# langfod/Zonos

Hardware: AMD Instinct MI355X
Metric: audio-sec/sec (RTF), Zonos-v0.1-transformer AR decode loop + DAC decode (higher is better)
Workload: dtype bf16; 1 GPU; Zonos-v0.1-transformer bf16, batch=1 per GPU, 10 s target audio (861 frames, 868 decode steps + prefill of 25 positions, EOS suppressed), greedy, cfg_scale 2; weights=seeded synthetic (zonos_amd/synth.py), parallelism=dp1 (utterance sharding, no data-path collective)

## Files before the change

### zonos_amd/csrc/zn_api.hip

```cpp
#include "../../include/zonos_hip.h"
#include "zn_decode_kernels.h"
#include "zn_chain_kernel.h"
#include "zn_step_kernel.h"
#include "zn_prefill_kernels.h"
#include "zn_cond_kernels.h"
#include "zn_mamba_kernels.h"

#include <cmath>
#include <cstdio>
#include <cstdlib>
#include <cstring>
#include <mutex>
#include <string>
#include <vector>

static thread_local std::string g_create_err;
#define ZN_GRAPH_STEPS 8
#define ZN_G16_PART_BYTES ((size_t)8 << 20)
#define ZN_REARM_AFTER 4

struct StepPlan {
  enum Path { LAUNCHES, CHAIN, STACK } path = LAUNCHES;
  int nbk = 0;
  int attn_fused = 0;
// ... 536 lines not shown
struct PostAttnPlans { LinearPlan out, fc1; };
static PostAttnPlans plan_post_attention(zn_handle h, int rows) {
  const zn_config& c = h->cfg;
  const LinearEnv e = linear_env(h);
  PostAttnPlans pp;
  pp.out = plan_linear(e, PRO_NONE, EPI_RESID, rows, c.d_model, c.n_heads * h->hd, h->tune[ZN_TUNE_WG_OUT_PROJ], false, true, false);
  pp.fc1 = plan_linear(e, PRO_LN, EPI_SILU, rows, 2 * c.d_ff, c.d_model, h->tune[ZN_TUNE_WG_FC1], false, false, pp.out.writes_ln_stats);
  return pp;
}

static int layer_in_proj(zn_handle h, int li, bf16_t* x, bf16_t* kv, int max_len, const int* lengths, int rows, hipStream_t s) {
  return run_gemv<PRO_LN, EPI_ROPE_KV>(h, in_proj_args(h, h->layers[li], x, kv, max_len, lengths), rows, h->tune[ZN_TUNE_WG_IN_PROJ], s);
}

static int layer_post_attention(zn_handle h, int li, bf16_t* x, int rows, hipStream_t s, bf16_t* x1_copy = nullptr) {
  const zn_layer_weights& lw = h->layers[li];
  const PostAttnPlans pp = plan_post_attention(h, rows);
  int rc;
  GemvArgs o = out_proj_args(h, lw, h->o1, x, x);
  o.ln_part_out = h->ln_part;
  if (h->cfg.double_out_proj) {
    if ((rc = run_gemv<PRO_NONE, EPI_STORE>(h, out_proj_args(h, lw, h->o1, h->q, nullptr), rows, h->tune[ZN_TUNE_WG_OUT_PROJ], s))) return rc;
    o.x = h->q;
  }
  if ((rc = launch_linear<PRO_NONE, EPI_RESID>(h, pp.out, o, rows, s))) return rc;
  if (x1_copy) (void)hipMemcpyAsync(x1_copy, x, (size_t)rows * h->cfg.d_model * 2, hipMemcpyDeviceToDevice, s);
  if ((rc = launch_linear<PRO_LN, EPI_SILU>(h, pp.fc1, fc1_args(h, lw, x, pp.out.writes_ln_stats ? h->ln_part : nullptr), rows, s))) return rc;
  return run_gemv<PRO_NONE, EPI_RESID>(h, fc2_args(h, lw, x), rows, h->tune[ZN_TUNE_WG_FC2], s);
}

static int layer_decode(zn_handle h, int li, bf16_t* x, bf16_t* kv, int max_len, const int* lengths, const int* ext,
                        int ext_scalar, int rows, int attn_fused, hipStream_t s) {
  int rc;
  if ((rc = layer_in_proj(h, li, x, kv, max_len, lengths, rows, s))) return rc;
  if ((rc = run_attention(h, h->q, kv, max_len, lengths, ext, ext_scalar, h->o1, rows, attn_fused, s))) return rc;
  return layer_post_attention(h, li, x, rows, s);
}

static bf16_t* chain_x(zn_handle h, int li) { return (li & 1) ? h->ch_x2 : h->x; }

static bool chain_heads_fit(zn_handle h) {
  const int units = (h->cfg.n_codebooks * h->cfg.vocab_head + 1) / 2, ppw = (units + ZN_CH_GRID - 1) / ZN_CH_GRID;
  return ppw <= ZN_CH_CWAVES * 5 && ppw * 2 <= 64;
}

static int launch_chain(zn_handle h, int li, const std::vector<const void*>& kv_layers, int max_len, const int* lengths, hipStream_t s,
                        const bf16_t* xin = nullptr, bool with_heads = false) {
  const zn_config& c = h->cfg;
  const zn_layer_weights& lw = h->layers[li];
  const bool last = li + 1 >= c.n_layer;
  ChainArgs a{};
  a.W_out = (const bf16_t*)lw.out_proj; a.W_fc1 = (const bf16_t*)lw.fc1; a.W_fc2 = (const bf16_t*)lw.fc2;
  a.ln2_w = (const bf16_t*)lw.norm2_w; a.ln2_b = (const bf16_t*)lw.norm2_b; a.eps = c.norm_eps; a.F = c.d_ff;
  a.a = h->o1; a.xin = xin ? xin : chain_x(h, li); a.xout = chain_x(h, li + 1);
  a.g_y1 = h->ch_gy1; a.g_x1 = h->ch_gx1; a.g_x2 = h->ch_gx2; a.g_m = h->ch_gm;
  a.epoch = h->ch_epoch; a.tmo = &h->st->pad[0]; a.diag = h->ch_diag;
  a.dbg_pause = h->dbg_pause; a.stamp_layer = li;
  a.stamps = h->ch_stamps ? h->ch_stamps + (size_t)li * 32 : nullptr;
  if (!last) {
    const zn_layer_weights& nx = h->layers[li + 1];
    a.W_in = (const bf16_t*)nx.in_proj; a.lnn_w = (const bf16_t*)nx.norm_w; a.lnn_b = (const bf16_t*)nx.norm_b;
    a.nqkv = (c.n_heads + 2 * c.n_heads_kv) * h->hd;
    a.q_out = h->q; a.kv = (bf16_t*)kv_layers[li + 1]; a.rope = h->rope; a.lengths = lengths;
    a.max_len = max_len; a.hd = h->hd; a.n_heads = c.n_heads; a.n_heads_kv = c.n_heads_kv; a.rope_positions = c.rope_positions;
  }
  const bool heads = last && with_heads;
  if (heads) {
    a.W_in = (const bf16_t*)h->heads; a.lnn_w = (const bf16_t*)h->norm_f_w; a.lnn_b = (const bf16_t*)h->norm_f_b;
    a.nqkv = c.n_codebooks * c.vocab_head; a.heads_out = h->logits_raw;
  }
  const dim3 grid(ZN_CH_GRID), block(ZN_CH_THREADS);
  if (h->ch_variant == 1) {
    if (heads) hipLaunchKernelGGL((chain_kernel<4, 1, 8, 4, 5>), grid, block, ZN_CH_DYN_LDS, s, a);
    else if (last) hipLaunchKernelGGL((chain_kernel<4, 1, 8, 4, 0>), grid, block, ZN_CH_DYN_LDS, s, a);
    else hipLaunchKernelGGL((chain_kernel<4, 1, 8, 4, 2>), grid, block, ZN_CH_DYN_LDS, s, a);
  } else {
    if (heads) hipLaunchKernelGGL((chain_kernel<1, 1, 2, 1, 5>), grid, block, ZN_CH_DYN_LDS, s, a);
    else if (last) hipLaunchKernelGGL((chain_kernel<1, 1, 2, 1, 0>), grid, block, ZN_CH_DYN_LDS, s, a);
    else hipLaunchKernelGGL((chain_kernel<1, 1, 2, 1, 1>), grid, block, ZN_CH_DYN_LDS, s, a);
  }
  return ZN_OK;
}

#define ZN_SK_T1 4, 2, 10, 5, 6, 6
#define ZN_SK_T2 4, 2, 11, 6, 7, 8
#define ZN_SK_T3 4, 2, 13, 7, 8, 12
static int stack_variant_of(int mode) { return mode <= 6 ? 1 : mode <= 8 ? 2 : 3; }
template <int R, int NCH, int T_OUT, int T_FC1, int T_FC2, int T_IN, int NBV>
static bool stack_variant_ok(zn_handle h, int natt) {
  const zn_config& c = h->cfg;
  const int nsw = ZN_CH_GRID - natt;
  if (nsw < 64) return false;
  auto most = [&](int units) { return (units + nsw - 1) / nsw; };
  const int nqkv = (c.n_heads + 2 * c.n_heads_kv) * h->hd;
  const int p_out = most(c.d_model / 2), p_fc1 = 2 * most(c.d_ff / 2), p_qkv = most((nqkv + 1) / 2), p_hd = most((c.n_codebooks * c.vocab_head + 1) / 2);
  if (p_out > ZN_SK_CW * T_OUT || p_out > T_FC2 || p_fc1 > ZN_SK_CW * T_FC1 || p_qkv > ZN_SK_CW * T_IN || p_hd > ZN_SK_CW * T_IN) return false;
  if (p_qkv > 10) return false;
  if (p_out * 2 > 64 || p_out * 4 > 64 || p_fc1 > 64 || p_qkv * 2 > 64 || p_hd * 2 > 64 || nqkv % 2) return false;
  const void* fn = R == 1 ? (const void*)step_r1_kernel<NCH, T_OUT, T_FC1, T_FC2, T_IN, NBV> : (const void*)step_kernel<NCH, T_OUT, T_FC1, T_FC2, T_IN, NBV>;
  int dev = 0, n_cus = 0, per_cu = 0;
  if (hipGetDevice(&dev) != hipSuccess || hipDeviceGetAttribute(&n_cus, hipDeviceAttributeMultiprocessorCount, dev) != hipSuccess) { (void)hipGetLastError(); return false; }
  if (hipFuncSetAttribute(fn, hipFuncAttributeMaxDynamicSharedMemorySize, ZN_SK_DYN_LDS) != hipSuccess) { (void)hipGetLastError(); return false; }
  if (hipOccupancyMaxActiveBlocksPerMultiprocessor(&per_cu, fn, ZN_SK_THREADS, ZN_SK_DYN_LDS) != hipSuccess) { (void)hipGetLastError(); return false; }
  hipFuncAttributes fa{};
  if (hipFuncGetAttributes(&fa, fn) != hipSuccess) { (void)hipGetLastError(); return false; }
  return per_cu >= 1 && n_cus >= ZN_CH_GRID && fa.localSizeBytes == 0;
}
static bool stack_shapes_ok(zn_handle h) {
  const zn_config& c = h->cfg;
  if (h->ch_variant != 1 || h->hd != 128 || c.n_heads_kv < 1 || c.n_heads != 4 * c.n_heads_kv) return false;
  const int npairs = 2 * c.n_heads_kv, nkvh = c.n_heads_kv;
  h->stackv_ok[1] = stack_variant_ok<2, ZN_SK_T1>(h, npairs * 6);
  h->stackv_ok[2] = stack_variant_ok<2, ZN_SK_T2>(h, npairs * 8);
  h->stackv_ok[3] = stack_variant_ok<2, ZN_SK_T3>(h, npairs * ZN_SK_KB_MAXNB);
  h->stackv1_ok[1] = stack_variant_ok<1, ZN_SK_T1>(h, nkvh * 6);
  h->stackv1_ok[2] = stack_variant_ok<1, ZN_SK_T2>(h, nkvh * 8);
  h->stackv1_ok[3] = stack_variant_ok<1, ZN_SK_T3>(h, nkvh * ZN_SK_KB_MAXNB);
  h->stack1_ok = h->stackv1_ok[1];
  return h->stackv_ok[1];
}
static bool persist_allowed(zn_handle h) { return h->tune[ZN_TUNE_PERSISTENT] != 2 && !h->demoted && h->persist_ok && !h->rows_unequal2 && !h->prefix_set; }
static bool persist_shape(zn_handle h, int rows) { return h->ch_variant != 0 && (rows == 2 || (rows == 1 && h->ch_variant == 1)); }
static bool persist_active(zn_handle h, int rows) { return persist_shape(h, rows) && persist_allowed(h); }
static int stack_blocks_for(zn_handle h, int rows, int keys_upper_bound) {
  if (h->tune[ZN_TUNE_WHOLE_STEP] == 2 || !(rows == 1 ? h->stack1_ok : h->stack_ok)) return -1;
  const int nb = keys_upper_bound <= 512 ? 1 : (keys_upper_bound + 511) / 512;
  return nb <= ZN_SK_KB_MAXNB && (rows == 1 ? h->stackv1_ok : h->stackv_ok)[stack_variant_of(nb)] ? nb : -1;
}
static int graph_slot_for(const StepPlan& p) { return p.path == StepPlan::STACK ? 8 + (p.run > 1 ? ZN_SK_KB_MAXNB + 1 : 0) + p.nbk : p.attn_fused + (p.run > 1 ? 4 : 0); }
static bool chain_allowed(zn_handle h, int rows) { return h->ch_variant != 0 && rows == 2 && persist_allowed(h); }
static StepPlan plan_blocks(zn_handle h, int rows, int keys) {
  StepPlan p;
  p.path = chain_allowed(h, rows) ? StepPlan::CHAIN : StepPlan::LAUNCHES; p.attn_fused = attn_fused_for(h, keys);
  return p;
}
static StepPlan plan_steps(zn_handle h, int steps_left) {
  const int rows = h->rows, keys = h->len_hi + 1, keys_run = h->len_hi + ZN_GRAPH_STEPS;
  const bool want_run = steps_left >= ZN_GRAPH_STEPS && h->tune[ZN_TUNE_GRAPH_RUNS] > 1;
  const bool tail_ok = h->cfg.arch == 0 && persist_active(h, rows) && h->batch <= 2;
  const int nb_run = tail_ok && want_run ? stack_blocks_for(h, rows, keys_run) : -1;
  const int nb_one = tail_ok ? stack_blocks_for(h, rows, keys) : -1;
  StepPlan p = plan_blocks(h, rows, keys);
  if (nb_run >= 0 || nb_one >= 0) {
    p.path = StepPlan::STACK; p.nbk = nb_run >= 0 ? nb_run : nb_one; p.run = nb_run >= 0 ? ZN_GRAPH_STEPS : 1;
  } else if (want_run && attn_fused_for(h, keys_run) == p.attn_fused) p.run = ZN_GRAPH_STEPS;
  p.fused_tail = tail_ok && p.path != StepPlan::LAUNCHES;
  p.graph_slot = graph_slot_for(p);
  return p;
}
static bool stack_pre(zn_handle h) { return h->tune[ZN_TUNE_STACK_PRE] != 2; }
static int launch_stack(zn_handle h, hipStream_t s, int rows, int nbk) {
  const zn_config& c = h->cfg;
  ChainArgs a{};
  a.eps = c.norm_eps; a.F = c.d_ff; a.nqkv = (c.n_heads + 2 * c.n_heads_kv) * h->hd;
  a.xin = h->x_emb; a.xout = h->x;
  a.g_y1 = h->ch_gy1; a.g_x1 = h->ch_gx1; a.g_x2 = h->ch_gx2; a.g_m = h->ch_gm; a.g_qkv = h->ch_gqkv; a.g_a = h->ch_ga;
  a.g_bmax = h->ch_gbmax; a.g_part = h->ch_gpart;
  a.epoch = h->ch_epoch; a.tmo = &h->st->pad[0]; a.diag = h->ch_diag;
  a.dbg_pause = h->dbg_pause;
  a.stamps = h->ch_stamps; a.stamp_layer = c.n_layer / 2;
  a.rope = h->rope; a.lengths = h->lengths; a.max_len = h->max_len; a.hd = h->hd; a.n_heads = c.n_heads; a.n_heads_kv = c.n_heads_kv;
  a.rope_positions = c.rope_positions;
  a.layers = h->stack_layers; a.n_layer = c.n_layer; a.q0 = h->q; a.scale = (float)(1.0 / std::sqrt((double)h->hd));
  a.heads_rows = c.n_codebooks * c.vocab_head; a.heads_out = h->logits_raw; a.trace = h->dbg_trace;
  const int mode = nbk, npairs = rows * c.n_heads_kv;
  a.natt = npairs * (mode < 1 ? 1 : mode);
  if (stack_pre(h)) {
    a.pre_W = (const bf16_t*)h->layers[0].in_proj; a.pre_ln_w = (const bf16_t*)h->layers[0].norm_w; a.pre_ln_b = (const bf16_t*)h->layers[0].norm_b;
    a.pre_kv = (bf16_t*)h->kv_layers[0];
  }
  const dim3 grid(ZN_CH_GRID), block(ZN_SK_THREADS);
  if (rows == 1) {
    switch (stack_variant_of(mode)) {
      case 1: hipLaunchKernelGGL((step_r1_kernel<ZN_SK_T1>), grid, block, ZN_SK_DYN_LDS, s, a); break;
      case 2: hipLaunchKernelGGL((step_r1_kernel<ZN_SK_T2>), grid, block, ZN_SK_DYN_LDS, s, a); break;
      default: hipLaunchKernelGGL((step_r1_kernel<ZN_SK_T3>), grid, block, ZN_SK_DYN_LDS, s, a); break;
    }
    return ZN_OK;
  }
// ... 1088 lines not shown
```

### zonos_amd/csrc/zn_step_kernel.h

```cpp
#pragma once
#include "zn_chain_kernel.h"
#include "zn_step_sched.h"

#define ZN_SK_THREADS 512
#define ZN_SK_CW 4
#ifndef ZN_SK_NBUF
#define ZN_SK_NBUF 3
#endif
#ifndef ZN_SK_PARK
#define ZN_SK_PARK 4
#endif
#ifndef ZN_SK_HELP
#define ZN_SK_HELP 0
#endif
#ifndef ZN_SK_HELP_AT
#define ZN_SK_HELP_AT 0
#endif
#ifndef ZN_SK_EARLY
#define ZN_SK_EARLY 0
#endif
#ifndef ZN_SK_MSWEEP_DELAY
#define ZN_SK_MSWEEP_DELAY 0
#endif
#ifndef ZN_SK_SWEEP_DELAY
#define ZN_SK_SWEEP_DELAY 32
#endif
#define ZN_SK_DYN_LDS (ZN_SK_CW * ZN_SK_PARK * 8192)
#ifndef ZN_SK_APOLL
#define ZN_SK_APOLL 1
#endif
#ifndef ZN_SK_XDELAY
#define ZN_SK_XDELAY 16
#endif
#ifndef ZN_SK_XDELAY_NB
#define ZN_SK_XDELAY_NB 5
#endif
#ifndef ZN_SK_PACE_MARGIN
#define ZN_SK_PACE_MARGIN 0
#endif
#ifndef ZN_SK_PACE_SHIFT
#define ZN_SK_PACE_SHIFT 2
#endif

#ifndef ZN_SK_PACE_CAP
#define ZN_SK_PACE_CAP 8192u
#endif
#define ZN_SK_LONG_WAIT 20000u
struct StepPacer {
  unsigned long long t_ref; unsigned prev;
  unsigned worst = 0, n_long = 0;
  ZN_DEVINL void start() { t_ref = __builtin_amdgcn_s_memrealtime(); }
  ZN_DEVINL void sleep() const {
#ifdef ZN_TIMING_STREAM_ONLY
    return;
#endif
    const unsigned long long until = t_ref + (ZN_SK_PACE_MARGIN > 0 ? (prev > ZN_SK_PACE_MARGIN ? prev - ZN_SK_PACE_MARGIN : 0u) : (prev - (prev >> ZN_SK_PACE_SHIFT)));
    while (__builtin_amdgcn_s_memrealtime() < until) __builtin_amdgcn_s_sleep(8);
  }
  ZN_DEVINL void done() {
    const unsigned long long d = __builtin_amdgcn_s_memrealtime() - t_ref;
    prev = d < ZN_SK_PACE_CAP ? (unsigned)d : ZN_SK_PACE_CAP;
    const unsigned du = d < 0xffffffffull ? (unsigned)d : 0xffffffffu;
    worst = du > worst ? du : worst;
    n_long += du > ZN_SK_LONG_WAIT ? 1u : 0u;
  }
  ZN_DEVINL void report(unsigned* diag, int lane) const {
    if (lane == 0 && diag) { if (worst > ZN_SK_LONG_WAIT / 2) atomicMax(diag + 8, worst); if (n_long) atomicAdd(diag + 9, n_long); }
  }
};
ZN_DEVINL void step_debug_pause(unsigned ticks) {
  const unsigned long long t0 = __builtin_amdgcn_s_memrealtime();
  while (__builtin_amdgcn_s_memrealtime() - t0 < ticks) __builtin_amdgcn_s_sleep(127);
}

#define ZN_SK_KB_MAXNB 12
#define ZN_SK_KB_PSZ 520
struct StepKbLds {
  float sc[4][512];
  float bm[8][4];
  float bmall[ZN_SK_KB_MAXNB][4];
  float accw[8][4][128];
  float l[8][4];
  __attribute__((aligned(16))) bf16_t p[4][512];
  __attribute__((aligned(16))) bf16_t q[4][128];
  __attribute__((aligned(16))) bf16_t knew[128], vnew[128];
  __attribute__((aligned(16))) bf16_t out[4][128];
};
static_assert(sizeof(StepKbLds) <= ZN_SK_DYN_LDS, "the key-block attention role's LDS fits the launch's dynamic LDS");

template <int CH, int DEPTH>
ZN_DEVINL void kb_combine_chunk(__amdgpu_buffer_rsrc_t rs_part, int voff, int loff, int j0, int nb, unsigned tag, const float (*bmall)[4], int g,
                                float& tot0, float& tot1, float& lt, float& mprev, int* tmo, int lane, SweepWho who) {
  constexpr int PSZ8 = ZN_SK_KB_PSZ * 8;
  u32x4 pv[DEPTH][CH];
  u32x2 pl[DEPTH][CH];
  auto issue = [&](auto DC) {
    constexpr int d = decltype(DC)::value;
#pragma unroll
    for (int j = 0; j < CH; ++j) {
      const int jo = min(j0 + j, nb - 1) * PSZ8;
      pv[d][j] = ld_sc1_16(rs_part, voff + jo);
      pl[d][j] = ld_sc1_8(rs_part, loff + jo);
    }
  };
  zn_static_for<0, DEPTH>([&](auto DC) { issue(DC); });
  SpinBound sb; sb.begin();
  int got = -1;
  while (got < 0) {
    zn_static_for<0, DEPTH>([&](auto DC) {
      constexpr int d = decltype(DC)::value;
// ... 212 lines not shown
      const int g = tid >> 7, d = tid & 127;
      float v = 0.f, l = 0.f;
#pragma unroll
      for (int w = 0; w < NW; ++w) v += S.accw[w][g][d];
#pragma unroll
      for (int w = 0; w < NW; ++w) l += S.l[w][g];
      if (nb == 1) S.out[g][d] = f2bf(__fmul_rn(v, 1.0f / l));
      else {
        unsigned long long* pp = a.g_part + ((size_t)pair * MAXNB + jb) * PSZ;
        st_granule(pp + g * 128 + d, tag, __float_as_uint(v));
        if (d == 0) st_granule(pp + G * 128 + g, tag, __float_as_uint(l));
      }
    }
    if (nb == 1) __syncthreads();
    stamp(5);
    if (wave < 4 && (nb == 1 || jb == 0)) {
      const int p = tid, g = p >> 6, dp = p & 63;
      unsigned o;
      if (nb == 1) o = *(const unsigned*)&S.out[g][2 * dp];
      else {
        const int voff = ((pair * MAXNB) * PSZ + g * 128 + 2 * dp) * 8, loff = ((pair * MAXNB) * PSZ + G * 128 + g) * 8;
        float tot0 = 0.f, tot1 = 0.f, lt = 0.f, mprev = -INFINITY;
        const SweepWho who{(8u << 8) | (unsigned)li, a.diag};
        if (ZN_SK_XDELAY > 0 && nb >= ZN_SK_XDELAY_NB) __builtin_amdgcn_s_sleep(ZN_SK_XDELAY);
        if (nb <= 2) kb_combine_chunk<2, ZN_SK_APOLL>(rs_part, voff, loff, 0, nb, tag, S.bmall, g, tot0, tot1, lt, mprev, a.tmo, lane, who);
        else if (nb <= 4) kb_combine_chunk<4, 2>(rs_part, voff, loff, 0, nb, tag, S.bmall, g, tot0, tot1, lt, mprev, a.tmo, lane, who);
        else {
#pragma unroll
          for (int j0 = 0; j0 < NBV; j0 += 6)
            if (j0 < nb) kb_combine_chunk<6, 1>(rs_part, voff, loff, j0, nb, tag, S.bmall, g, tot0, tot1, lt, mprev, a.tmo, lane, who);
        }
        const float inv = 1.0f / lt;
        o = pack2(__fmul_rn(tot0, inv), __fmul_rn(tot1, inv));
      }
      st_granule(a.g_a + (size_t)ar * (D / 2) + ((kvh * G + g) * HD) / 2 + dp, tag, o);
      if (a.trace) *(unsigned*)(a.trace + ((size_t)(8 * li + 1) * R + ar) * D + (kvh * G + g) * HD + 2 * dp) = o;
    }
    if (a.trace && jb == 0 && wave == ZN_SK_CW)
      *(u32x4*)(a.trace + ((size_t)(8 * li + 2) * R + ar) * D + (kvh * G + (lane >> 4)) * HD + (lane & 15) * 8) = *(const u32x4*)&S.q[lane >> 4][(lane & 15) * 8];
    stamp(6);
    if (li + 1 < a.n_layer) {
      int opq = 0;
      asm volatile("" : "+v"(opq));
      issue_kv(a.layers[li + 1].kv, opq, lane);
    }
    pace.start();
  }
  if (wave == ZN_SK_CW) pace.report(a.diag, lane_in);
}

template <int R, int NCH, int T_OUT, int T_FC1, int T_FC2, int T_IN, int NBV>
ZN_DEVINL void step_body(const ChainArgs& a) {
  static_assert(R == 1 || R == 2, "one or two activation rows");
  constexpr int D = NCH * 512, CW = ZN_SK_CW;
  constexpr int NS = 2 * T_OUT + T_FC1 + T_FC2 + T_IN;
  constexpr int NOPS = 5;
  constexpr int MASK = ZN_CH_DEFER_MASK;
  constexpr int NB = ZN_SK_NBUF, P = ZN_SK_PARK;
  constexpr int NL = NS - T_OUT;
  static_assert(T_IN > 0 && NCH == 4, "step_kernel: d_model 2048, head size 128");
  static_assert(P >= T_OUT && NB >= 2 && P + NB <= NL, "op 0's tiles are parked (op 1 reads them again); the prefetch stays inside the block");
  const int tid = threadIdx.x, lane = tid & 63, wave = __builtin_amdgcn_readfirstlane(tid >> 6);
  const int c = blockIdx.x;
  const int F = a.F;
  const unsigned tag0 = ld_sc1_u32(a.epoch);
  extern __shared__ __attribute__((aligned(16))) unsigned char zn_dyn_lds[];
  const int natt = a.natt;
  if (c < natt) {
    step_attention_kb_role<NBV, R>(a, *reinterpret_cast<StepKbLds*>(zn_dyn_lds), tag0, c, wave, lane);
    return;
  }
  __shared__ __attribute__((aligned(16))) bf16_t s_act[R * D];
  __shared__ float s_res[2][64][2][R];
  __shared__ __attribute__((aligned(16))) bf16_t s_ln[4 * D];
  const int sc = c - natt, NSW = (int)gridDim.x - natt;
  auto split = [&](int U, int& n, int& start) { const int base = U / NSW, extra = U % NSW; n = base + (sc < extra ? 1 : 0); start = sc * base + min(sc, extra); };
  int n_out, s_out, ng1, sg1;
  split(D / 2, n_out, s_out);
  split(F / 2, ng1, sg1);
  const int n_fc1 = 2 * ng1, s_fc1 = 2 * sg1;
  int n_qkv, s_qkv, n_hd, s_hd;
  split((a.nqkv + 1) / 2, n_qkv, s_qkv);
  split((a.heads_rows + 1) / 2, n_hd, s_hd);
  constexpr int NBAR = 14;
  __shared__ int s_pf[2];
  constexpr int NPT = 5;
  const bool pre = a.pre_W != nullptr;
  if (tid < 2) s_pf[tid] = 0;
  __syncthreads();

  using SC = StepSched<T_OUT, T_FC1, T_FC2, T_IN, NB, P, ZN_SK_HELP, MASK, ZN_SK_EARLY>;
  auto op_of = [](int s) constexpr { return SC::op_of(s); };
  auto first_of = [](int op) constexpr { return SC::first_of(op); };

  constexpr int L_F2 = SC::L_F2;
  constexpr int NH = ZN_SK_HELP;
  static_assert(NH >= 0 && NH <= T_OUT && NH < T_FC1 - (P - T_OUT), "helper tiles take the slots of op 0's tiles");
  constexpr int NREG = SC::NREG;
  auto slot_of_load = [](int l) constexpr { return SC::slot_of_load(l); };
  struct WT { u32x4 a[NCH], b[NCH]; };
  struct LW { const bf16_t *out, *fc1, *fc2, *in; };
  auto tile_of = [&](const LW& Lr, int rows_in, int n_in, int s_in, int s, int w, bool& ok, const bf16_t*& pa, const bf16_t*& pb, int& ridx) {
    const int op = op_of(s), t = s - first_of(op);
    if (op == 3) {
      const int qt = w, j = t;
      ok = j < n_out;
      const int u = s_out + (ok ? j : 0);
      pa = Lr.fc2 + (size_t)(2 * u) * (4 * D) + qt * D + lane * 8;
      pb = pa + 4 * D;
      ridx = j * 4 + qt;
      return;
    }
    const int j = w + CW * t;
    const int n = op <= 1 ? n_out : op == 2 ? n_fc1 : n_in;
    const int st = op <= 1 ? s_out : op == 2 ? s_fc1 : s_in;
    ok = j < n;
    const int u = st + (ok ? j : 0);
    ridx = j;
    if (op <= 1) { pa = Lr.out + (size_t)(2 * u) * D + lane * 8; pb = pa + D; }
    else if (op == 2) { pa = Lr.fc1 + (size_t)u * D + lane * 8; pb = pa + (size_t)F * D; }
    else { pa = Lr.in + (size_t)(2 * u) * D + lane * 8; pb = (2 * u + 1 < rows_in) ? pa + D : pa; }
  };
  auto park_of = [&](int w) { return reinterpret_cast<u32x4*>(zn_dyn_lds) + (size_t)w * (P * 2 * NCH * 64) + lane; };

  if (wave >= CW + 2) {
    const int hw = wave - (CW + 2);
    WT hb[2 * (NH > 0 ? NH : 1)];
    if (pre) {
      WT pt[NPT];
#pragma unroll
      for (int t = 0; t < NPT; ++t) {
        const int j = hw + 2 * t;
        if (j < n_qkv) {
          const int u = s_qkv + j;
          const bf16_t* pa = a.pre_W + (size_t)(2 * u) * D + lane * 8;
          const bf16_t* pb = (2 * u + 1 < a.nqkv) ? pa + D : pa;
#pragma unroll
          for (int c2 = 0; c2 < NCH; ++c2) { pt[t].a[c2] = ld_nt16(pa + c2 * 512); pt[t].b[c2] = ld_nt16(pb + c2 * 512); }
        }
      }
      while (__hip_atomic_load(&s_pf[0], __ATOMIC_ACQUIRE, __HIP_MEMORY_SCOPE_WORKGROUP) < R) __builtin_amdgcn_s_sleep(1);
      u32x4 xr[NCH][R];
#pragma unroll
      for (int c2 = 0; c2 < NCH; ++c2)
#pragma unroll
        for (int r = 0; r < R; ++r) xr[c2][r] = *(const u32x4*)&s_act[r * D + (c2 * 64 + lane) * 8];
#pragma unroll
      for (int t = 0; t < NPT; ++t) {
        const int j = hw + 2 * t;
        if (j < n_qkv) {
          float accA[R] = {}, accB[R] = {};
#pragma unroll
          for (int c2 = 0; c2 < NCH; ++c2) {
#pragma unroll
            for (int r = 0; r < R; ++r) { accA[r] = dot8(pt[t].a[c2], xr[c2][r], accA[r]); accB[r] = dot8(pt[t].b[c2], xr[c2][r], accB[r]); }
          }
#pragma unroll
          for (int r = 0; r < R; ++r) { accA[r] = wave_sum(accA[r]); accB[r] = wave_sum(accB[r]); }
          if (lane == 0) {
#pragma unroll
            for (int r = 0; r < R; ++r) { s_res[0][j][0][r] = accA[r]; s_res[0][j][1][r] = accB[r]; }
          }
        }
      }
      if (lane == 0) __hip_atomic_fetch_add(&s_pf[1], 1, __ATOMIC_RELEASE, __HIP_MEMORY_SCOPE_WORKGROUP);
    }
#pragma unroll 1
    for (int li = 0; li < a.n_layer; ++li) {
      const LW Lr{a.layers[li].W_out, a.layers[li].W_fc1, a.layers[li].W_fc2, a.layers[li].W_in};
      auto hload = [&]() {
        if constexpr (NH > 0) {
          zn_static_for<0, 2 * NH>([&](auto IC) {
            constexpr int i = decltype(IC)::value, cwi = i / NH, hh = i % NH;
            bool ok; const bf16_t *pa, *pb; int ridx;
            tile_of(Lr, a.nqkv, 0, 0, slot_of_load(L_F2 - NH + hh), 2 * hw + cwi, ok, pa, pb, ridx);
            if (ok) {
#pragma unroll
              for (int c2 = 0; c2 < NCH; ++c2) { hb[i].a[c2] = ld_nt16g(pa + c2 * 512); hb[i].b[c2] = ld_nt16g(pb + c2 * 512); }
            }
          });
        }
      };
      {
        const bf16_t* p0 = hw == 0 ? a.layers[li].ln2_w : a.layers[li].lnn_w;
        const bf16_t* p1 = hw == 0 ? a.layers[li].ln2_b : a.layers[li].lnn_b;
#pragma unroll
        for (int c2 = 0; c2 < NCH; ++c2) {
          *(u32x4*)&s_ln[(2 * hw) * D + (c2 * 64 + lane) * 8] = ld16g(p0 + (c2 * 64 + lane) * 8);
          *(u32x4*)&s_ln[(2 * hw + 1) * D + (c2 * 64 + lane) * 8] = ld16g(p1 + (c2 * 64 + lane) * 8);
        }
      }
      if constexpr (ZN_SK_HELP_AT == 0) hload();
      __syncthreads();
      if constexpr (ZN_SK_HELP_AT == 1) hload();
      __syncthreads();
      __syncthreads();
      if constexpr (ZN_SK_HELP_AT == 2) hload();
      __syncthreads();
      __syncthreads();
      if constexpr (NH > 0) {
        zn_static_for<0, 2 * NH>([&](auto IC) {
          constexpr int i = decltype(IC)::value, cwi = i / NH, hh = i % NH;
          bool ok; const bf16_t *pa, *pb; int ridx;
          tile_of(Lr, a.nqkv, 0, 0, slot_of_load(L_F2 - NH + hh), 2 * hw + cwi, ok, pa, pb, ridx);
          if (ok) {
            u32x4* pk = park_of(2 * hw + cwi);
#pragma unroll
            for (int c2 = 0; c2 < NCH; ++c2) { pk[(hh * 2 * NCH + c2) * 64] = hb[i].a[c2]; pk[(hh * 2 * NCH + NCH + c2) * 64] = hb[i].b[c2]; }
          }
        });
      }
#pragma unroll
      for (int b = 5; b < NBAR; ++b) __syncthreads();
    }
    return;
  }

  if (wave < CW) {
    WT bufs[NB];
    u32x4* park = park_of(wave);
    static_assert(CW == 4, "fc2 splits K over the four compute waves");
    const bool st_on = a.stamps && sc == 0 && wave == 0 && lane == 0;
#pragma unroll 1
    for (int li = 0; li < a.n_layer; ++li) {
      const LW Lr{a.layers[li].W_out, a.layers[li].W_fc1, a.layers[li].W_fc2, a.layers[li].W_in};
      const bool last = li + 1 == a.n_layer;
      const int rows_in = last ? a.heads_rows : a.nqkv;
      const int n_in = last ? n_hd : n_qkv, s_in = last ? s_hd : s_qkv;
      const unsigned tag = tag0 + 1u + (unsigned)li;
      const bool stamped = st_on && li == a.stamp_layer;
      auto cstamp = [&](int i) { if (stamped) a.stamps[40 + i] = __builtin_amdgcn_s_memrealtime(); };
      auto tile = [&](int s, bool& ok, const bf16_t*& pa, const bf16_t*& pb, int& ridx) { tile_of(Lr, rows_in, n_in, s_in, s, wave, ok, pa, pb, ridx); };
      auto load_into = [&](auto LC, auto BC) {
        constexpr int l = decltype(LC)::value, b = decltype(BC)::value;
        if constexpr (l >= 0 && l < NL) {
          bool ok; const bf16_t *pa, *pb; int ridx;
          tile(slot_of_load(l), ok, pa, pb, ridx);
          if (ok) {
            WT& w = bufs[b];
#ifdef ZN_TIMING_HANDOFFS_ONLY
#pragma unroll
            for (int c2 = 0; c2 < NCH; ++c2) { w.a[c2] = u32x4{0, 0, 0, 0}; w.b[c2] = u32x4{0, 0, 0, 0}; }
#else
#pragma unroll
            for (int c2 = 0; c2 < NCH; ++c2) { w.a[c2] = ld_nt16g(pa + c2 * 512); w.b[c2] = ld_nt16g(pb + c2 * 512); }
#endif
          }
        }
      };
      auto reg_req = [&](auto KC) {
        constexpr int k = decltype(KC)::value;
        if constexpr (k >= 0 && k < NREG) load_into(std::integral_constant<int, SC::nth_reg(k >= 0 && k < NREG ? k : 0)>{}, std::integral_constant<int, ((k >= 0 ? k : 0) + P) % NB>{});
      };
      u32x4 xr[NCH][R];
      auto process = [&](int s, const WT& w) {
        bool ok; const bf16_t *pa, *pb; int ridx;
        tile(s, ok, pa, pb, ridx);
        if (!ok) return;
        float accA[R] = {}, accB[R] = {};
#pragma unroll
        for (int c2 = 0; c2 < NCH; ++c2) {
#pragma unroll
          for (int r = 0; r < R; ++r) { accA[r] = dot8(w.a[c2], xr[c2][r], accA[r]); accB[r] = dot8(w.b[c2], xr[c2][r], accB[r]); }
        }
#pragma unroll
        for (int r = 0; r < R; ++r) { accA[r] = wave_sum(accA[r]); accB[r] = wave_sum(accB[r]); }
        if (lane == 0) {
          const int par = op_of(s) & 1;
#pragma unroll
          for (int r = 0; r < R; ++r) { s_res[par][ridx][0][r] = accA[r]; s_res[par][ridx][1][r] = accB[r]; }
        }
      };
      cstamp(0);
      zn_static_for<0, NB>([&](auto IC) {
        constexpr int i = decltype(IC)::value;
        if constexpr (i < P) load_into(std::integral_constant<int, i>{}, std::integral_constant<int, i % NB>{});
        else reg_req(std::integral_constant<int, i - P>{});
      });
      zn_static_for<0, P>([&](auto LC) {
        constexpr int l = decltype(LC)::value;
        bool ok; const bf16_t *pa, *pb; int ridx;
        tile(slot_of_load(l), ok, pa, pb, ridx);
        if (ok) {
          const WT& w = bufs[l % NB];
#pragma unroll
          for (int c2 = 0; c2 < NCH; ++c2) { park[(l * 2 * NCH + c2) * 64] = w.a[c2]; park[(l * 2 * NCH + NCH + c2) * 64] = w.b[c2]; }
        }
        constexpr int i = l + NB;
        if constexpr (i < P) load_into(std::integral_constant<int, i>{}, std::integral_constant<int, i % NB>{});
        else reg_req(std::integral_constant<int, i - P>{});
      });
      cstamp(1);
      zn_static_for<0, NS>([&](auto SC) {
        constexpr int s = decltype(SC)::value;
        constexpr int op = op_of(s);
        if constexpr (s == first_of(op)) {
          if constexpr (op > 0) {
            __syncthreads();
            __syncthreads();
            zn_static_for<SC::first_of(op - 1), SC::first_of(op)>([&](auto QC) {
              constexpr int q = decltype(QC)::value;
              if constexpr (SC::raise_late(q)) reg_req(std::integral_constant<int, SC::raised_by(q)>{});
            });
          }
          if constexpr (op == 3) {
            u32x4 dat[NCH * R];
            const int mbase = (wave * (D / 2) + lane * 4) * 8;
            if constexpr (ZN_SK_MSWEEP_DELAY > 0) __builtin_amdgcn_s_sleep(ZN_SK_MSWEEP_DELAY);
            sweep_granules_at<NCH * R>(zn_rsrc(a.g_m), [&](int i) { return mbase + ((i % R) * (2 * D) + (i / R) * 256) * 8; }, tag, dat, a.tmo, lane,
                                       SweepWho{(3u << 8) | (unsigned)li, a.diag});
#pragma unroll
            for (int c2 = 0; c2 < NCH; ++c2)
#pragma unroll
              for (int r = 0; r < R; ++r) xr[c2][r] = dat[c2 * R + r];
          } else {
            __syncthreads();
#pragma unroll
            for (int c2 = 0; c2 < NCH; ++c2)
#pragma unroll
              for (int r = 0; r < R; ++r) xr[c2][r] = *(const u32x4*)&s_act[r * D + (c2 * 64 + lane) * 8];
          }
          cstamp(2 + 2 * op);
        }
        constexpr int l = SC::load_of_slot(s);
        if constexpr (SC::src_of(l) != 0) {
          bool ok; const bf16_t *pa, *pb; int ridx;
          tile(s, ok, pa, pb, ridx);
          if (ok) {
            constexpr int sl = SC::slot_of(l);
            WT w;
#pragma unroll
            for (int c2 = 0; c2 < NCH; ++c2) { w.a[c2] = park[(sl * 2 * NCH + c2) * 64]; w.b[c2] = park[(sl * 2 * NCH + NCH + c2) * 64]; }
            process(s, w);
          }
        } else {
          constexpr int k = SC::regk(l);
          process(s, bufs[(k + P) % NB]);
          if constexpr (SC::raise_now(s)) reg_req(std::integral_constant<int, SC::raised_by(s)>{});
        }
        if constexpr (s + 1 == NS || op_of(s + 1 < NS ? s + 1 : s) != op) cstamp(3 + 2 * op);
      });
      __syncthreads();
      __syncthreads();
    }
    return;
  }

  const int myr = wave - CW;
  if constexpr (R == 1) {
    if (myr >= R) {
#pragma unroll 1
      for (int li = 0; li < a.n_layer; ++li)
#pragma unroll
        for (int b = 0; b < NBAR; ++b) __syncthreads();
      return;
    }
  }
  const bool epi = myr == 0;
  u32x4 g[NCH];
  const int ij = lane >> 1, ir = lane & 1;
  const bool it_out = epi && ij < n_out && ir < R;
  const int u_out = s_out + (it_out ? ij : 0);
  unsigned resid = 0;
  if (it_out) resid = *(const unsigned*)(a.xin + (size_t)ir * D + 2 * u_out);
  const int nq = a.n_heads * a.hd, nk = a.n_heads_kv * a.hd;
  const bool it_qkv = epi && ij < n_qkv && ir < R;
  const int u_qkv = s_qkv + (it_qkv ? ij : 0);
  int pos = 0; float cs = 1.f, sn = 0.f;
  if (it_qkv) {
    pos = a.lengths[ir];
    const int rowA = 2 * u_qkv;
    if (rowA < nq + nk) {
      const int i = (rowA % a.hd) >> 1;
      const int p = pos < a.rope_positions ? pos : a.rope_positions - 1;
      const float2 c2v = *(const float2*)(a.rope + ((size_t)p * (a.hd >> 1) + i) * 2);
      cs = c2v.x; sn = c2v.y;
    }
  }
  int goff[NCH];
#pragma unroll
  for (int c2 = 0; c2 < NCH; ++c2) goff[c2] = (myr * (D / 2) + (c2 * 64 + lane) * 4) * 8;
  unsigned x1own = 0;
  if (pre) {
    u32x4 lw[NCH], lb[NCH];
#pragma unroll
    for (int c2 = 0; c2 < NCH; ++c2) {
      g[c2] = ld16(a.xin + (size_t)myr * D + (c2 * 64 + lane) * 8);
      lw[c2] = ld16(a.pre_ln_w + (c2 * 64 + lane) * 8);
      lb[c2] = ld16(a.pre_ln_b + (c2 * 64 + lane) * 8);
    }
    chain_layernorm_row<NCH>(g, lw, lb, a.eps);
#pragma unroll
    for (int c2 = 0; c2 < NCH; ++c2) *(u32x4*)&s_act[myr * D + (c2 * 64 + lane) * 8] = g[c2];
    if (lane == 0) __hip_atomic_fetch_add(&s_pf[0], 1, __ATOMIC_RELEASE, __HIP_MEMORY_SCOPE_WORKGROUP);
    while (__hip_atomic_load(&s_pf[1], __ATOMIC_ACQUIRE, __HIP_MEMORY_SCOPE_WORKGROUP) < 2) __builtin_amdgcn_s_sleep(1);
    if (it_qkv) {
      const int rowA = 2 * u_qkv;
      const float x0 = bfround(s_res[0][ij][0][ir]), x1 = bfround(s_res[0][ij][1][ir]);
      unsigned packed;
      if (rowA < nq + nk) {
        float re, im;
        zn_rope_pair(x0, x1, cs, sn, re, im);
        packed = pack2(re, im);
      } else packed = pack2(x0, x1);
      st_granule(a.g_qkv + (size_t)ir * (a.nqkv / 2) + u_qkv, tag0, packed);
      if (rowA >= nq && pos < a.max_len) {
        const int which = rowA < nq + nk ? 0 : 1, colk = rowA - nq - which * nk;
        *(unsigned*)(a.pre_kv + (((size_t)ir * a.max_len + pos) * 2 + which) * nk + colk) = packed;
      }
    }
  }
  StepPacer pace{0ull, 0u};
  pace.start();
#pragma unroll 1
  for (int li = 0; li < a.n_layer; ++li) {
    const StackLayer& Lr = a.layers[li];
    const bool last = li + 1 == a.n_layer;
    const unsigned tag = tag0 + 1u + (unsigned)li;
    const bool stamped = a.stamps && li == a.stamp_layer && epi && sc == 0 && lane == 0;
    int nst = 0;
    auto stamp = [&]() { if (stamped) a.stamps[nst] = __builtin_amdgcn_s_memrealtime(); ++nst; };
    stamp();
    int opq = 0;
    asm volatile("" : "+v"(opq));
    const int irq = ir + opq, uoq = u_out + opq, uqq = u_qkv + opq;
    pace.sleep();
    stamp();
    sweep_granules<NCH>(zn_rsrc(a.g_a), goff, tag, g, a.tmo, lane, SweepWho{(6u << 8) | (unsigned)li, a.diag});
    pace.done();
#pragma unroll
    for (int c2 = 0; c2 < NCH; ++c2) *(u32x4*)&s_act[myr * D + (c2 * 64 + lane) * 8] = g[c2];
    __syncthreads();
    stamp();
    zn_static_for<0, NOPS>([&](auto OC) {
      constexpr int op = decltype(OC)::value;
      constexpr int par = op & 1;
      __syncthreads();
      stamp();
      if constexpr (op == 0) {
        if (it_out) st_granule(a.g_y1 + (size_t)irq * (D / 2) + uoq, tag, pack2(s_res[par][ij][0][ir], s_res[par][ij][1][ir]));
      } else if constexpr (op == 1) {
        if (it_out) {
          x1own = pack2(lo_f(resid) + bfround(s_res[par][ij][0][ir]), hi_f(resid) + bfround(s_res[par][ij][1][ir]));
          st_granule(a.g_x1 + (size_t)irq * (D / 2) + uoq, tag, x1own);
        }
      } else if constexpr (op == 2) {
        const bool on = lane < n_fc1;
        const int jj = on ? lane : 0;
        const float y = bfround(s_res[par][jj][0][myr]), gt = bfround(s_res[par][jj][1][myr]);
        const float sg = bfround(gt / (1.0f + expf(-gt)));
        const unsigned mine = (unsigned)f2bf(y * sg);
        const unsigned nbv = (unsigned)__shfl_down((int)mine, 1);
        if (on && (lane & 1) == 0) st_granule(a.g_m + (size_t)(myr + opq) * (F / 2) + ((s_fc1 + lane) >> 1), tag, mine | (nbv << 16));
      } else if constexpr (op == 3) {
        if (it_out) {
          const float vA = ((s_res[par][ij * 4 + 0][0][ir] + s_res[par][ij * 4 + 1][0][ir]) + s_res[par][ij * 4 + 2][0][ir]) + s_res[par][ij * 4 + 3][0][ir];
          const float vB = ((s_res[par][ij * 4 + 0][1][ir] + s_res[par][ij * 4 + 1][1][ir]) + s_res[par][ij * 4 + 2][1][ir]) + s_res[par][ij * 4 + 3][1][ir];
          const unsigned o = pack2(lo_f(x1own) + bfround(vA), hi_f(x1own) + bfround(vB));
          st_granule(a.g_x2 + (size_t)irq * (D / 2) + uoq, tag, o);
          if (last) *(unsigned*)(a.xout + (size_t)irq * D + 2 * uoq) = o;
          if (a.trace) *(unsigned*)(a.trace + ((size_t)(8 * li) * R + irq) * D + 2 * uoq) = o;
          resid = o;
        }
      } else {
        if (last) {
          if (epi && ij < n_hd && ir < R) {
            const int u = s_hd + ij;
            a.heads_out[(size_t)irq * a.heads_rows + 2 * u] = bfround(s_res[par][ij][0][ir]);
            if (2 * u + 1 < a.heads_rows) a.heads_out[(size_t)irq * a.heads_rows + 2 * u + 1] = bfround(s_res[par][ij][1][ir]);
          }
        } else if (it_qkv) {
          const int rowA = 2 * u_qkv;
          const float x0 = bfround(s_res[par][ij][0][ir]), x1 = bfround(s_res[par][ij][1][ir]);
          unsigned packed;
          if (rowA < nq + nk) {
            float re, im;
            zn_rope_pair(x0, x1, cs, sn, re, im);
            packed = pack2(re, im);
          } else packed = pack2(x0, x1);
          st_granule(a.g_qkv + (size_t)irq * (a.nqkv / 2) + uqq, tag, packed);
          if (rowA >= nq && pos < a.max_len) {
            const int which = rowA < nq + nk ? 0 : 1, colk = rowA - nq - which * nk;
            *(unsigned*)(Lr.kv_next + (((size_t)irq * a.max_len + pos) * 2 + which) * nk + colk) = packed;
          }
        }
      }
      __syncthreads();
      stamp();
      if constexpr (op + 1 < NOPS) {
        if constexpr (op != 2) {
          if constexpr (ZN_SK_SWEEP_DELAY > 0) __builtin_amdgcn_s_sleep(ZN_SK_SWEEP_DELAY);
          sweep_granules<NCH>(zn_rsrc(op == 0 ? a.g_y1 : op == 1 ? a.g_x1 : a.g_x2), goff, tag, g, a.tmo, lane,
                              SweepWho{((op == 0 ? 1u : op == 1 ? 2u : 4u) << 8) | (unsigned)li, a.diag});
          stamp();
          if constexpr (op == 1 || op == 3) {
            u32x4 lw[NCH], lb[NCH];
#pragma unroll
            for (int c2 = 0; c2 < NCH; ++c2) {
              lw[c2] = *(const u32x4*)&s_ln[(op == 1 ? 0 : 2) * D + (c2 * 64 + lane) * 8];
              lb[c2] = *(const u32x4*)&s_ln[(op == 1 ? 1 : 3) * D + (c2 * 64 + lane) * 8];
            }
            chain_layernorm_row<NCH>(g, lw, lb, a.eps);
          }
#pragma unroll
          for (int c2 = 0; c2 < NCH; ++c2) *(u32x4*)&s_act[myr * D + (c2 * 64 + lane) * 8] = g[c2];
          __syncthreads();
        } else stamp();
        stamp();
      }
    });
    if (a.dbg_pause && li == 2) step_debug_pause(a.dbg_pause);
    pace.start();
  }
  pace.report(a.diag, lane);
  if (epi && sc == 0 && lane == 0) st_sc1_u32(a.epoch, tag0 + 1u + (unsigned)a.n_layer);
}

#define ZN_SK_DETACH_ARGS(a, a_in) \
  ChainArgs a = a_in;                \
  asm volatile("" : "+s"(a.max_len), "+s"(a.hd), "+s"(a.n_heads), "+s"(a.n_heads_kv), "+s"(a.rope_positions), "+s"(a.F), "+s"(a.nqkv), "+s"(a.natt), "+s"(a.dbg_pause))

template <int NCH, int T_OUT, int T_FC1, int T_FC2, int T_IN, int NBV>
__global__ __launch_bounds__(ZN_SK_THREADS) void step_kernel(ChainArgs a_in) {
  ZN_SK_DETACH_ARGS(a, a_in);
  step_body<2, NCH, T_OUT, T_FC1, T_FC2, T_IN, NBV>(a);
}

template <int NCH, int T_OUT, int T_FC1, int T_FC2, int T_IN, int NBV>
__global__ __launch_bounds__(ZN_SK_THREADS) void step_r1_kernel(ChainArgs a_in) {
  ZN_SK_DETACH_ARGS(a, a_in);
  step_body<1, NCH, T_OUT, T_FC1, T_FC2, T_IN, NBV>(a);
}
```

Measured before the change: 13.51 audio-sec/sec.

## Use six compute waves in the stack step kernel, dropping helper waves

The streaming workgroup's default wave split moves from four compute waves plus two helper waves to six compute waves. The pre-contraction and layernorm-parameter staging that helpers used to do move onto the compute waves. Because fc2 splits K four ways, the gathered fc2 input is now staged in LDS, reusing the parked-tile space with the parking depth halved, and shared by all six waves at the cost of extra barriers. Tile-count templates are retuned for the wider split. The aim is more concurrent weight streaming per CU, at the risk of less prefetch depth and more synchronization.

Measured after the change: 13.86 audio-sec/sec, median of 6. 1.03x the previous value.

```diff
diff --git a/zonos_amd/csrc/zn_api.hip b/zonos_amd/csrc/zn_api.hip
--- a/zonos_amd/csrc/zn_api.hip
+++ b/zonos_amd/csrc/zn_api.hip
@@ -642,9 +642,15 @@
   return ZN_OK;
 }
 
+#if ZN_SK_CW == 6
+#define ZN_SK_T1 4, 1, 7, 4, 4, 6
+#define ZN_SK_T2 4, 1, 8, 4, 5, 8
+#define ZN_SK_T3 4, 2, 9, 5, 5, 12
+#else
 #define ZN_SK_T1 4, 2, 10, 5, 6, 6
 #define ZN_SK_T2 4, 2, 11, 6, 7, 8
 #define ZN_SK_T3 4, 2, 13, 7, 8, 12
+#endif
 static int stack_variant_of(int mode) { return mode <= 6 ? 1 : mode <= 8 ? 2 : 3; }
 template <int R, int NCH, int T_OUT, int T_FC1, int T_FC2, int T_IN, int NBV>
 static bool stack_variant_ok(zn_handle h, int natt) {
@@ -654,7 +660,7 @@
   auto most = [&](int units) { return (units + nsw - 1) / nsw; };
   const int nqkv = (c.n_heads + 2 * c.n_heads_kv) * h->hd;
   const int p_out = most(c.d_model / 2), p_fc1 = 2 * most(c.d_ff / 2), p_qkv = most((nqkv + 1) / 2), p_hd = most((c.n_codebooks * c.vocab_head + 1) / 2);
-  if (p_out > ZN_SK_CW * T_OUT || p_out > T_FC2 || p_fc1 > ZN_SK_CW * T_FC1 || p_qkv > ZN_SK_CW * T_IN || p_hd > ZN_SK_CW * T_IN) return false;
+  if (p_out > ZN_SK_CW * T_OUT || 4 * p_out > ZN_SK_CW * T_FC2 || p_fc1 > ZN_SK_CW * T_FC1 || p_qkv > ZN_SK_CW * T_IN || p_hd > ZN_SK_CW * T_IN) return false;
   if (p_qkv > 10) return false;
   if (p_out * 2 > 64 || p_out * 4 > 64 || p_fc1 > 64 || p_qkv * 2 > 64 || p_hd * 2 > 64 || nqkv % 2) return false;
   const void* fn = R == 1 ? (const void*)step_r1_kernel<NCH, T_OUT, T_FC1, T_FC2, T_IN, NBV> : (const void*)step_kernel<NCH, T_OUT, T_FC1, T_FC2, T_IN, NBV>;
diff --git a/zonos_amd/csrc/zn_step_kernel.h b/zonos_amd/csrc/zn_step_kernel.h
--- a/zonos_amd/csrc/zn_step_kernel.h
+++ b/zonos_amd/csrc/zn_step_kernel.h
@@ -3,12 +3,15 @@
 #include "zn_step_sched.h"
 
 #define ZN_SK_THREADS 512
-#define ZN_SK_CW 4
+#ifndef ZN_SK_CW
+#define ZN_SK_CW 6
+#endif
+#define ZN_SK_HELPERS (8 - (ZN_SK_CW + 2))
 #ifndef ZN_SK_NBUF
 #define ZN_SK_NBUF 3
 #endif
 #ifndef ZN_SK_PARK
-#define ZN_SK_PARK 4
+#define ZN_SK_PARK (ZN_SK_CW == 4 ? 4 : 2)
 #endif
 #ifndef ZN_SK_HELP
 #define ZN_SK_HELP 0
@@ -26,6 +29,9 @@
 #define ZN_SK_SWEEP_DELAY 32
 #endif
 #define ZN_SK_DYN_LDS (ZN_SK_CW * ZN_SK_PARK * 8192)
+static_assert(ZN_SK_CW == 4 || ZN_SK_CW == 6, "4 compute waves + 2 helper waves, or 6 compute waves");
+static_assert(ZN_SK_DYN_LDS + 26 * 1024 <= 160 * 1024, "parked tiles + the streaming role's static LDS fit a CU");
+static_assert(ZN_SK_CW == 4 || ZN_SK_DYN_LDS >= 2 * 4 * 2048 * 2, "fc2's input [2][4 d_model] is staged in the parked tiles' LDS");
 #ifndef ZN_SK_APOLL
 #define ZN_SK_APOLL 1
 #endif
@@ -404,9 +410,11 @@
   int n_qkv, s_qkv, n_hd, s_hd;
   split((a.nqkv + 1) / 2, n_qkv, s_qkv);
   split((a.heads_rows + 1) / 2, n_hd, s_hd);
-  constexpr int NBAR = 14;
+  constexpr bool MLDS = CW != 4;
+  constexpr int NBAR = 14 + (MLDS ? 1 : 0);
   __shared__ int s_pf[2];
-  constexpr int NPT = 5;
+  constexpr int NPW = ZN_SK_HELPERS > 0 ? ZN_SK_HELPERS : CW;
+  constexpr int NPT = (10 + NPW - 1) / NPW;
   const bool pre = a.pre_W != nullptr;
   if (tid < 2) s_pf[tid] = 0;
   __syncthreads();
@@ -418,6 +426,7 @@
   constexpr int L_F2 = SC::L_F2;
   constexpr int NH = ZN_SK_HELP;
   static_assert(NH >= 0 && NH <= T_OUT && NH < T_FC1 - (P - T_OUT), "helper tiles take the slots of op 0's tiles");
+  static_assert(NH == 0 || ZN_SK_HELPERS == 2, "helper tiles need the two helper waves");
   constexpr int NREG = SC::NREG;
   auto slot_of_load = [](int l) constexpr { return SC::slot_of_load(l); };
   struct WT { u32x4 a[NCH], b[NCH]; };
@@ -425,7 +434,7 @@
   auto tile_of = [&](const LW& Lr, int rows_in, int n_in, int s_in, int s, int w, bool& ok, const bf16_t*& pa, const bf16_t*& pb, int& ridx) {
     const int op = op_of(s), t = s - first_of(op);
     if (op == 3) {
-      const int qt = w, j = t;
+      const int i = w + CW * t, qt = i & 3, j = i >> 2;
       ok = j < n_out;
       const int u = s_out + (ok ? j : 0);
       pa = Lr.fc2 + (size_t)(2 * u) * (4 * D) + qt * D + lane * 8;
@@ -445,48 +454,50 @@
   };
   auto park_of = [&](int w) { return reinterpret_cast<u32x4*>(zn_dyn_lds) + (size_t)w * (P * 2 * NCH * 64) + lane; };
 
-  if (wave >= CW + 2) {
+  auto pre_contract = [&](int pw) {
+    WT pt[NPT];
+#pragma unroll
+    for (int t = 0; t < NPT; ++t) {
+      const int j = pw + NPW * t;
+      if (j < n_qkv) {
+        const int u = s_qkv + j;
+        const bf16_t* pa = a.pre_W + (size_t)(2 * u) * D + lane * 8;
+        const bf16_t* pb = (2 * u + 1 < a.nqkv) ? pa + D : pa;
+#pragma unroll
+        for (int c2 = 0; c2 < NCH; ++c2) { pt[t].a[c2] = ld_nt16(pa + c2 * 512); pt[t].b[c2] = ld_nt16(pb + c2 * 512); }
+      }
+    }
+    while (__hip_atomic_load(&s_pf[0], __ATOMIC_ACQUIRE, __HIP_MEMORY_SCOPE_WORKGROUP) < R) __builtin_amdgcn_s_sleep(1);
+    u32x4 xr[NCH][R];
+#pragma unroll
+    for (int c2 = 0; c2 < NCH; ++c2)
+#pragma unroll
+      for (int r = 0; r < R; ++r) xr[c2][r] = *(const u32x4*)&s_act[r * D + (c2 * 64 + lane) * 8];
+#pragma unroll
+    for (int t = 0; t < NPT; ++t) {
+      const int j = pw + NPW * t;
+      if (j < n_qkv) {
+        float accA[R] = {}, accB[R] = {};
+#pragma unroll
+        for (int c2 = 0; c2 < NCH; ++c2) {
+#pragma unroll
+          for (int r = 0; r < R; ++r) { accA[r] = dot8(pt[t].a[c2], xr[c2][r], accA[r]); accB[r] = dot8(pt[t].b[c2], xr[c2][r], accB[r]); }
+        }
+#pragma unroll
+        for (int r = 0; r < R; ++r) { accA[r] = wave_sum(accA[r]); accB[r] = wave_sum(accB[r]); }
+        if (lane == 0) {
+#pragma unroll
+          for (int r = 0; r < R; ++r) { s_res[0][j][0][r] = accA[r]; s_res[0][j][1][r] = accB[r]; }
+        }
+      }
+    }
+    if (lane == 0) __hip_atomic_fetch_add(&s_pf[1], 1, __ATOMIC_RELEASE, __HIP_MEMORY_SCOPE_WORKGROUP);
+  };
+
+  if (ZN_SK_HELPERS > 0 && wave >= CW + 2) {
     const int hw = wave - (CW + 2);
     WT hb[2 * (NH > 0 ? NH : 1)];
-    if (pre) {
-      WT pt[NPT];
-#pragma unroll
-      for (int t = 0; t < NPT; ++t) {
-        const int j = hw + 2 * t;
-        if (j < n_qkv) {
-          const int u = s_qkv + j;
-          const bf16_t* pa = a.pre_W + (size_t)(2 * u) * D + lane * 8;
-          const bf16_t* pb = (2 * u + 1 < a.nqkv) ? pa + D : pa;
-#pragma unroll
-          for (int c2 = 0; c2 < NCH; ++c2) { pt[t].a[c2] = ld_nt16(pa + c2 * 512); pt[t].b[c2] = ld_nt16(pb + c2 * 512); }
-        }
-      }
-      while (__hip_atomic_load(&s_pf[0], __ATOMIC_ACQUIRE, __HIP_MEMORY_SCOPE_WORKGROUP) < R) __builtin_amdgcn_s_sleep(1);
-      u32x4 xr[NCH][R];
-#pragma unroll
-      for (int c2 = 0; c2 < NCH; ++c2)
-#pragma unroll
-        for (int r = 0; r < R; ++r) xr[c2][r] = *(const u32x4*)&s_act[r * D + (c2 * 64 + lane) * 8];
-#pragma unroll
-      for (int t = 0; t < NPT; ++t) {
-        const int j = hw + 2 * t;
-        if (j < n_qkv) {
-          float accA[R] = {}, accB[R] = {};
-#pragma unroll
-          for (int c2 = 0; c2 < NCH; ++c2) {
-#pragma unroll
-            for (int r = 0; r < R; ++r) { accA[r] = dot8(pt[t].a[c2], xr[c2][r], accA[r]); accB[r] = dot8(pt[t].b[c2], xr[c2][r], accB[r]); }
-          }
-#pragma unroll
-          for (int r = 0; r < R; ++r) { accA[r] = wave_sum(accA[r]); accB[r] = wave_sum(accB[r]); }
-          if (lane == 0) {
-#pragma unroll
-            for (int r = 0; r < R; ++r) { s_res[0][j][0][r] = accA[r]; s_res[0][j][1][r] = accB[r]; }
-          }
-        }
-      }
-      if (lane == 0) __hip_atomic_fetch_add(&s_pf[1], 1, __ATOMIC_RELEASE, __HIP_MEMORY_SCOPE_WORKGROUP);
-    }
+    if (pre) pre_contract(hw);
 #pragma unroll 1
     for (int li = 0; li < a.n_layer; ++li) {
       const LW Lr{a.layers[li].W_out, a.layers[li].W_fc1, a.layers[li].W_fc2, a.layers[li].W_in};
@@ -541,7 +552,7 @@
   if (wave < CW) {
     WT bufs[NB];
     u32x4* park = park_of(wave);
-    static_assert(CW == 4, "fc2 splits K over the four compute waves");
+    if constexpr (ZN_SK_HELPERS == 0) { if (pre) pre_contract(wave); }
     const bool st_on = a.stamps && sc == 0 && wave == 0 && lane == 0;
 #pragma unroll 1
     for (int li = 0; li < a.n_layer; ++li) {
@@ -575,10 +586,20 @@
         if constexpr (k >= 0 && k < NREG) load_into(std::integral_constant<int, SC::nth_reg(k >= 0 && k < NREG ? k : 0)>{}, std::integral_constant<int, ((k >= 0 ? k : 0) + P) % NB>{});
       };
       u32x4 xr[NCH][R];
+      auto m_lds = [&](int qt) { return reinterpret_cast<u32x4*>(zn_dyn_lds) + (size_t)qt * (NCH * R * 64) + lane; };
       auto process = [&](int s, const WT& w) {
         bool ok; const bf16_t *pa, *pb; int ridx;
         tile(s, ok, pa, pb, ridx);
         if (!ok) return;
+        if constexpr (MLDS) {
+          if (op_of(s) == 3) {
+            const u32x4* mq = m_lds(ridx & 3);
+#pragma unroll
+            for (int c2 = 0; c2 < NCH; ++c2)
+#pragma unroll
+              for (int r = 0; r < R; ++r) xr[c2][r] = mq[(c2 * R + r) * 64];
+          }
+        }
         float accA[R] = {}, accB[R] = {};
 #pragma unroll
         for (int c2 = 0; c2 < NCH; ++c2) {
@@ -594,11 +615,25 @@
         }
       };
       cstamp(0);
+      u32x4 lnp[NCH];
+      if constexpr (ZN_SK_HELPERS == 0) {
+        if (wave < 4) {
+          const bf16_t* lp = wave == 0 ? a.layers[li].ln2_w : wave == 1 ? a.layers[li].ln2_b : wave == 2 ? a.layers[li].lnn_w : a.layers[li].lnn_b;
+#pragma unroll
+          for (int c2 = 0; c2 < NCH; ++c2) lnp[c2] = ld16g(lp + (c2 * 64 + lane) * 8);
+        }
+      }
       zn_static_for<0, NB>([&](auto IC) {
         constexpr int i = decltype(IC)::value;
         if constexpr (i < P) load_into(std::integral_constant<int, i>{}, std::integral_constant<int, i % NB>{});
         else reg_req(std::integral_constant<int, i - P>{});
       });
+      if constexpr (ZN_SK_HELPERS == 0) {
+        if (wave < 4) {
+#pragma unroll
+          for (int c2 = 0; c2 < NCH; ++c2) *(u32x4*)&s_ln[wave * D + (c2 * 64 + lane) * 8] = lnp[c2];
+        }
+      }
       zn_static_for<0, P>([&](auto LC) {
         constexpr int l = decltype(LC)::value;
         bool ok; const bf16_t *pa, *pb; int ridx;
@@ -626,15 +661,21 @@
             });
           }
           if constexpr (op == 3) {
-            u32x4 dat[NCH * R];
-            const int mbase = (wave * (D / 2) + lane * 4) * 8;
-            if constexpr (ZN_SK_MSWEEP_DELAY > 0) __builtin_amdgcn_s_sleep(ZN_SK_MSWEEP_DELAY);
-            sweep_granules_at<NCH * R>(zn_rsrc(a.g_m), [&](int i) { return mbase + ((i % R) * (2 * D) + (i / R) * 256) * 8; }, tag, dat, a.tmo, lane,
-                                       SweepWho{(3u << 8) | (unsigned)li, a.diag});
-#pragma unroll
-            for (int c2 = 0; c2 < NCH; ++c2)
-#pragma unroll
-              for (int r = 0; r < R; ++r) xr[c2][r] = dat[c2 * R + r];
+            if (!MLDS || wave < 4) {
+              u32x4 dat[NCH * R];
+              const int mbase = (wave * (D / 2) + lane * 4) * 8;
+              if constexpr (ZN_SK_MSWEEP_DELAY > 0) __builtin_amdgcn_s_sleep(ZN_SK_MSWEEP_DELAY);
+              sweep_granules_at<NCH * R>(zn_rsrc(a.g_m), [&](int i) { return mbase + ((i % R) * (2 * D) + (i / R) * 256) * 8; }, tag, dat, a.tmo, lane,
+                                         SweepWho{(3u << 8) | (unsigned)li, a.diag});
+#pragma unroll
+              for (int c2 = 0; c2 < NCH; ++c2)
+#pragma unroll
+                for (int r = 0; r < R; ++r) {
+                  if constexpr (MLDS) m_lds(wave)[(c2 * R + r) * 64] = dat[c2 * R + r];
+                  else xr[c2][r] = dat[c2 * R + r];
+                }
+            }
+            if constexpr (MLDS) __syncthreads();
           } else {
             __syncthreads();
 #pragma unroll
@@ -715,7 +756,7 @@
 #pragma unroll
     for (int c2 = 0; c2 < NCH; ++c2) *(u32x4*)&s_act[myr * D + (c2 * 64 + lane) * 8] = g[c2];
     if (lane == 0) __hip_atomic_fetch_add(&s_pf[0], 1, __ATOMIC_RELEASE, __HIP_MEMORY_SCOPE_WORKGROUP);
-    while (__hip_atomic_load(&s_pf[1], __ATOMIC_ACQUIRE, __HIP_MEMORY_SCOPE_WORKGROUP) < 2) __builtin_amdgcn_s_sleep(1);
+    while (__hip_atomic_load(&s_pf[1], __ATOMIC_ACQUIRE, __HIP_MEMORY_SCOPE_WORKGROUP) < NPW) __builtin_amdgcn_s_sleep(1);
     if (it_qkv) {
       const int rowA = 2 * u_qkv;
       const float x0 = bfround(s_res[0][ij][0][ir]), x1 = bfround(s_res[0][ij][1][ir]);
@@ -827,7 +868,10 @@
 #pragma unroll
           for (int c2 = 0; c2 < NCH; ++c2) *(u32x4*)&s_act[myr * D + (c2 * 64 + lane) * 8] = g[c2];
           __syncthreads();
-        } else stamp();
+        } else {
+          if constexpr (MLDS) __syncthreads();
+          stamp();
+        }
         stamp();
       }
     });
```
